# V2AI/Det3D

Measured on NVIDIA H100. Metric: point-clouds/sec SECOND SpMiddleFHD @20k pts, higher is better.
Workload: dtype f32

## Files before the change

### det3d_b200/csrc/spconv16_sm90.cu

```cuda
#include "epilogue16.cuh"

namespace d3b {

constexpr int kOsTileM = 128;
constexpr int kOsKc = 64;
constexpr int kOsABytes = kOsTileM * 128;

template <int COUT, int PLANES = 2>
struct OsCfg {
  static constexpr int kSlotHalves = 2 * COUT * kOsKc;
  static constexpr int kBBytes = PLANES * COUT * 128;
  static constexpr int kStageBytes = PLANES * kOsABytes + kBBytes;
  static constexpr int kStages = COUT >= 128 ? 3 : 4;
  static constexpr int kGroups = kStages;
  static constexpr int kMathWarps = 8;
  static constexpr int kGatherWarp0 = kMathWarps;
  static constexpr int kGroupThreads = 64;
  static constexpr int kThreads = 32 * (kGatherWarp0 + 2 * kGroups);
  static constexpr int kPassN = COUT >= 128 ? 64 : COUT;
  static constexpr int kSmemBytes = kStages * kStageBytes + 1024  + 256  + 32 * kOsTileM * 4;
};

template <int PLANES>
__device__ __forceinline__ bool epilogue16(float (&v)[16], const Epi16& e, size_t row_off, int col, __half* out_hi,
                                           __half* out_lo, float* out_f32) {
#pragma unroll
  for (int q = 0; q < 16; ++q) v[q] *= e.acc_scale;
  if (e.bias) {
#pragma unroll
    for (int q = 0; q < 16; q += 4) {
      const float4 b = __ldg(reinterpret_cast<const float4*>(e.bias + col + q));
      v[q] += b.x; v[q + 1] += b.y; v[q + 2] += b.z; v[q + 3] += b.w;
    }
  }
  if (e.scale) {
#pragma unroll
    for (int q = 0; q < 16; q += 4) {
      const float4 s = __ldg(reinterpret_cast<const float4*>(e.scale + col + q));
      const float4 t = __ldg(reinterpret_cast<const float4*>(e.shift + col + q));
      v[q] = fmaf(v[q], s.x, t.x); v[q + 1] = fmaf(v[q + 1], s.y, t.y);
      v[q + 2] = fmaf(v[q + 2], s.z, t.z); v[q + 3] = fmaf(v[q + 3], s.w, t.w);
    }
  }
  if (e.res_hi) {
#pragma unroll
    for (int q = 0; q < 16; q += 8) {
      if constexpr (PLANES == 2) {
        const uint4 h = __ldg(reinterpret_cast<const uint4*>(e.res_hi + row_off + col + q));
        const uint4 l = __ldg(reinterpret_cast<const uint4*>(e.res_lo + row_off + col + q));
        const uint32_t hw[4] = {h.x, h.y, h.z, h.w}, lw[4] = {l.x, l.y, l.z, l.w};
#pragma unroll
        for (int j = 0; j < 4; ++j) {
          const float2 fh = __half22float2(*reinterpret_cast<const __half2*>(&hw[j]));
          const float2 fl = __half22float2(*reinterpret_cast<const __half2*>(&lw[j]));
          v[q + 2 * j] += fh.x + fl.x;
          v[q + 2 * j + 1] += fh.y + fl.y;
        }
      } else {
        const uint4 h = __ldg(reinterpret_cast<const uint4*>(e.res_hi + row_off + col + q));
        const uint32_t hw[4] = {h.x, h.y, h.z, h.w};
#pragma unroll
        for (int j = 0; j < 4; ++j) {
          const float2 fh = __half22float2(*reinterpret_cast<const __half2*>(&hw[j]));
          v[q + 2 * j] += fh.x;
          v[q + 2 * j + 1] += fh.y;
        }
      }
    }
  }
  bool ovf = false;
  if (e.relu) {
#pragma unroll
    for (int q = 0; q < 16; ++q) v[q] = fmaxf(v[q], 0.f);
  }
  if (out_hi && PLANES == 2) {
    uint32_t hi[8], lo[8];
#pragma unroll
    for (int q = 0; q < 16; q += 2) ovf |= split_pack2(v[q], v[q + 1], hi[q >> 1], lo[q >> 1]);
    uint4* ph = reinterpret_cast<uint4*>(out_hi + row_off + col);
    uint4* pl = reinterpret_cast<uint4*>(out_lo + row_off + col);
    ph[0] = make_uint4(hi[0], hi[1], hi[2], hi[3]);
    ph[1] = make_uint4(hi[4], hi[5], hi[6], hi[7]);
    pl[0] = make_uint4(lo[0], lo[1], lo[2], lo[3]);
    pl[1] = make_uint4(lo[4], lo[5], lo[6], lo[7]);
  }
  if (out_hi && PLANES == 1) {
    uint32_t hi[8];
#pragma unroll
    for (int q = 0; q < 16; q += 2) {
      hi[q >> 1] = pack_half2(__float2half_rn(v[q]), __float2half_rn(v[q + 1]));
      ovf |= f16_out_of_range(v[q]) | f16_out_of_range(v[q + 1]);
    }
    uint4* ph = reinterpret_cast<uint4*>(out_hi + row_off + col);
    ph[0] = make_uint4(hi[0], hi[1], hi[2], hi[3]);
    ph[1] = make_uint4(hi[4], hi[5], hi[6], hi[7]);
  }
  if (out_f32) {
    float4* pf = reinterpret_cast<float4*>(out_f32 + row_off + col);
#pragma unroll
    for (int q = 0; q < 16; q += 4) pf[q >> 2] = make_float4(v[q], v[q + 1], v[q + 2], v[q + 3]);
  }
  return ovf;
}

template <int PLANES>
__device__ __forceinline__ bool epilogue2(float v0, float v1, const Epi16& e, size_t row_off, int col, __half* out_hi,
                                          __half* out_lo, float* out_f32) {
  v0 *= e.acc_scale;
  v1 *= e.acc_scale;
  v0 = fmaf(v0, e.corr, v0);
  v1 = fmaf(v1, e.corr, v1);
  if (e.bias) {
    const float2 b = __ldg(reinterpret_cast<const float2*>(e.bias + col));
    v0 += b.x; v1 += b.y;
  }
  if (e.scale) {
    const float2 s = __ldg(reinterpret_cast<const float2*>(e.scale + col));
    const float2 t = __ldg(reinterpret_cast<const float2*>(e.shift + col));
    v0 = fmaf(v0, s.x, t.x); v1 = fmaf(v1, s.y, t.y);
  }
  if (e.res_hi) {
    const float2 r = load_pair16<PLANES>(e.res_hi, e.res_lo, row_off + col);
    v0 += r.x;
    v1 += r.y;
  }
  if (e.relu) { v0 = fmaxf(v0, 0.f); v1 = fmaxf(v1, 0.f); }
  bool ovf = false;
  if (out_hi) ovf = store_pair16<PLANES>(v0, v1, out_hi, out_lo, row_off + col);
  if (out_f32) *reinterpret_cast<float2*>(out_f32 + row_off + col) = make_float2(v0, v1);
  return ovf;
}

__host__ __device__ inline int os16_pack(int c_in, int k_vol) {
  return k_vol > 1 && (c_in == 16 || c_in == 32) ? kOsKc / c_in : 1;
}
__device__ __forceinline__ unsigned int os16_slot_mask(unsigned int offset_mask, int pack) {
  if (pack == 1) return offset_mask;
  unsigned int r = 0u;
  const unsigned int grp = (1u << pack) - 1u;
  for (int p = 0; p * pack < 32; ++p) r |= ((offset_mask >> (p * pack)) & grp) ? (1u << p) : 0u;
  return r;
}

template <int COUT, int PLANES>
__device__ __forceinline__ void spconv_os16_body(
    const __half* __restrict__ in_hi, const __half* __restrict__ in_lo, const int* __restrict__ nbr,
    const unsigned int* __restrict__ tile_mask, const int* __restrict__ n_out_p, int out_cap, int c_in, int n_kb, int pack,
    int k_vol, const __half* __restrict__ packed, const Epi16& epi, __half* __restrict__ out_hi, __half* __restrict__ out_lo,
    float* __restrict__ out_f32, int* __restrict__ overflow) {
  using Cfg = OsCfg<COUT, PLANES>;
  extern __shared__ uint8_t smem_raw[];
  const uint32_t smem_base = (smem_u32(smem_raw) + 1023u) & ~1023u;
  uint8_t* smem_gen = smem_raw + (smem_base - smem_u32(smem_raw));
  const uint32_t bar_base = smem_base + Cfg::kStages * Cfg::kStageBytes;
  auto full_bar = [&](int s) { return bar_base + 8u * s; };
  auto empty_bar = [&](int s) { return bar_base + 8u * (Cfg::kStages + s); };
  const uint32_t nbr_bar = bar_base + 8u * (2 * Cfg::kStages);
  int* koff_s = reinterpret_cast<int*>(smem_gen + Cfg::kStages * Cfg::kStageBytes + 128);
  int* nbr_s = reinterpret_cast<int*>(smem_gen + Cfg::kStages * Cfg::kStageBytes + 256);

  D3B_CTA_MARK(0, epi.seq);
  pdl_launch_dependents();
  const int warp = threadIdx.x >> 5, lane = threadIdx.x & 31;
  const int n_out = min(*n_out_p, out_cap);
  const int n_tiles = (n_out + kOsTileM - 1) / kOsTileM;
  const int c_eff = c_in * pack;

  if (threadIdx.x == 0) {
    for (int s = 0; s < Cfg::kStages; ++s) {
      mbar_init(full_bar(s), Cfg::kGroupThreads + 1);
      mbar_init(empty_bar(s), Cfg::kMathWarps);
    }
    mbar_init(nbr_bar, 1);
    asm volatile("fence.mbarrier_init.release.cluster;" ::: "memory");
  }
  __syncthreads();

  if (warp < Cfg::kMathWarps) {
    pdl_wait_prior_grid();
    const int wg = warp >> 2, wq = warp & 3;
    bool ovf = false;
    uint32_t it = 0;
    for (int tile = blockIdx.x; tile < n_tiles; tile += gridDim.x) {
      const unsigned int smask = os16_slot_mask(tile_mask[tile], pack);
      const int n_slots = __popc(smask) * n_kb;
      float acc[COUT / 2];
#pragma unroll
      for (int q = 0; q < COUT / 2; ++q) acc[q] = 0.f;
      for (int j = 0; j < n_slots; ++j, ++it) {
        const int kb = n_kb == 1 ? 0 : j % n_kb;
        const int s = it % Cfg::kStages;
        const uint32_t ph = (it / Cfg::kStages) & 1u;
        const int n_ks = min(kOsKc / 16, (c_eff - kb * kOsKc + 15) / 16);
        if (warp == 0 && lane == 0) D3B_STAMP(6, it);
        D3B_WAIT(full_bar(s), ph, 3);
        const uint32_t a_hi = smem_base + s * Cfg::kStageBytes + wg * 8192u;
        const uint32_t a_lo = a_hi + kOsABytes;
        const uint32_t b_hi = smem_base + s * Cfg::kStageBytes + PLANES * kOsABytes;
        const uint32_t b_lo = b_hi + COUT * 128;
#pragma unroll
        for (int np = 0; np < COUT / Cfg::kPassN; ++np) {
          float part[Cfg::kPassN / 2];
          const uint32_t nb = np * Cfg::kPassN * 128;
          gmma_fence();
#pragma unroll
          for (int ks = 0; ks < kOsKc / 16; ++ks) {
            const uint32_t adv = ks * 32;
            if constexpr (PLANES == 2) {
              wgmma_f16<Cfg::kPassN>(part, gmma_desc_sw128(a_lo + adv), gmma_desc_sw128(b_hi + nb + adv), ks > 0 ? 1u : 0u);
              wgmma_f16<Cfg::kPassN>(part, gmma_desc_sw128(a_hi + adv), gmma_desc_sw128(b_lo + nb + adv), 1u);
              wgmma_f16<Cfg::kPassN>(part, gmma_desc_sw128(a_hi + adv), gmma_desc_sw128(b_hi + nb + adv), 1u);
            } else {
              wgmma_f16<Cfg::kPassN>(part, gmma_desc_sw128(a_hi + adv), gmma_desc_sw128(b_hi + nb + adv), ks > 0 ? 1u : 0u);
            }
          }
          gmma_commit();
          gmma_wait();
          gmma_fence_regs(part);
#pragma unroll
          for (int q = 0; q < Cfg::kPassN / 2; ++q) acc[np * Cfg::kPassN / 2 + q] += part[q];
        }
        __syncwarp();
        if (lane == 0) mbar_arrive(empty_bar(s));
        if (warp == 0 && lane == 0) D3B_STAMP(7, it);
      }
#pragma unroll
      for (int h = 0; h < 2; ++h) {
        const int o = tile * kOsTileM + wg * 64 + wq * 16 + (lane >> 2) + 8 * h;
        if (o >= n_out) continue;
#pragma unroll
        for (int jn = 0; jn < COUT / 8; ++jn)
          ovf |= epilogue2<PLANES>(acc[4 * jn + 2 * h], acc[4 * jn + 2 * h + 1], epi, (size_t)o * COUT, jn * 8 + 2 * (lane & 3),
                           out_hi, out_lo, out_f32);
      }
    }
    if (ovf && overflow) atomicOr(overflow, 1);
  } else {
    const int gw = warp - Cfg::kGatherWarp0;
    const int group = gw >> 1, wq = gw & 1;
    const int g = lane >> 3, c = lane & 7;
    const bool issues_tma = (wq == 0 && lane == 0);
    const int ptid = threadIdx.x - 32 * Cfg::kGatherWarp0;
    const int cpo = 8 / pack;
    const int sub = c / cpo;
    const int c_src = c - sub * cpo;
    uint32_t it0 = 0;
    uint32_t tile_count = 0;
    const bool bulk_nbr = (out_cap & 3) == 0;
    for (int tile = blockIdx.x; tile < n_tiles; tile += gridDim.x) {
      const int row0 = tile * kOsTileM;
      const unsigned int mask = os16_slot_mask(tile_mask[tile], pack);
      const int n_off = __popc(mask);
      const int n_slots = n_off * n_kb;

      asm volatile("bar.sync 1, %0;" ::"r"(Cfg::kGroupThreads * Cfg::kGroups) : "memory");
      if (ptid < 32) {
        unsigned int m = mask;
        for (int t = ptid; t > 0; --t) m &= m - 1;
        const int k = __ffs(m) - 1;
        if (ptid < n_off) koff_s[ptid] = k;
        __syncwarp();
        const int rows = min(kOsTileM, out_cap - row0);
        const int e_slot = ptid / pack;
        const int k_src = ptid < n_off * pack ? koff_s[e_slot] * pack + (ptid - e_slot * pack) : k_vol;
        const bool valid = k_src < k_vol;
        const unsigned int vm = __ballot_sync(0xffffffffu, valid);
        if (bulk_nbr && vm != 0u && ptid == 0) mbar_arrive_expect_tx(nbr_bar, (uint32_t)(__popc(vm) * rows * 4));
        __syncwarp();
        if (bulk_nbr && valid)
          tma_bulk_g2s(smem_u32(nbr_s + ptid * kOsTileM), nbr + (size_t)k_src * out_cap + row0, (uint32_t)(rows * 4), nbr_bar);
      }
      if (bulk_nbr) {
        if (n_off > 0) D3B_WAIT(nbr_bar, tile_count & 1u, 5);
      } else {
        asm volatile("bar.sync 1, %0;" ::"r"(Cfg::kGroupThreads * Cfg::kGroups) : "memory");
#pragma unroll 8
        for (int idx = ptid; idx < n_off * pack * kOsTileM; idx += Cfg::kGroupThreads * Cfg::kGroups) {
          const int r = idx & 127, e = idx >> 7;
          const int k_src = koff_s[e / pack] * pack + e % pack;
          nbr_s[idx] = k_src < k_vol ? __ldg(nbr + (size_t)k_src * out_cap + min(row0 + r, out_cap - 1)) : -1;
        }
      }
      asm volatile("bar.sync 1, %0;" ::"r"(Cfg::kGroupThreads * Cfg::kGroups) : "memory");
      if (n_off > 0) ++tile_count;
      if (tile == (int)blockIdx.x) pdl_wait_prior_grid();

      for (int j = (int)((group + Cfg::kGroups - (it0 % Cfg::kGroups)) % Cfg::kGroups); j < n_slots; j += Cfg::kGroups) {
        const int n = j / n_kb, kb = j - n * n_kb;
        const int ch = pack > 1 ? c_src * 8 : kb * kOsKc + c * 8;
        const uint32_t it = it0 + (uint32_t)j;
        const int s = it % Cfg::kStages;
        const uint32_t ph = (it / Cfg::kStages) & 1u;
        if (issues_tma) D3B_STAMP(0, it);
        D3B_WAIT(empty_bar(s), ph ^ 1u, 1);
        if (issues_tma) D3B_STAMP(1, it);
        const uint32_t stage = smem_base + s * Cfg::kStageBytes;
        if (issues_tma) {
          mbar_arrive_expect_tx(full_bar(s), Cfg::kBBytes);
          tma_bulk_g2s(stage + PLANES * kOsABytes, packed + ((size_t)koff_s[n] * n_kb + kb) * Cfg::kSlotHalves, Cfg::kBBytes,
                       full_bar(s));
        }
        {
          const int row_base = wq * 64 + g * 16;
          const int4* idx4 = reinterpret_cast<const int4*>(nbr_s + (n * pack + sub) * kOsTileM + row_base);
          const bool col_live = pack > 1 ? koff_s[n] * pack + sub < k_vol : ch < c_in;
#pragma unroll
          for (int q4 = 0; q4 < 4; ++q4) {
            const int4 iv = idx4[q4];
            const int srcs[4] = {iv.x, iv.y, iv.z, iv.w};
#pragma unroll
            for (int u = 0; u < 4; ++u) {
              const int row = row_base + q4 * 4 + u;
              const bool live = srcs[u] >= 0 && col_live && row0 + row < n_out;
              const size_t off = live ? (size_t)srcs[u] * c_in + ch : 0;
              const uint32_t dst = stage + sw128_offset(row, c);
              cp_async16(dst, in_hi + off, live ? 16u : 0u);
              if constexpr (PLANES == 2) cp_async16(dst + kOsABytes, in_lo + off, live ? 16u : 0u);
            }
          }
        }
        if (issues_tma) D3B_STAMP(2, it);
        cp_async_wait_all();
        if (issues_tma) D3B_STAMP(3, it);
        fence_proxy_async();
        mbar_arrive(full_bar(s));
      }
      it0 += (uint32_t)n_slots;
    }
  }
  D3B_CTA_MARK(1, epi.seq);
}

template <int COUT>
__global__ void __launch_bounds__(OsCfg<COUT>::kThreads, 1)
spconv_os16_kernel(const __half* __restrict__ in_hi, const __half* __restrict__ in_lo, const int* __restrict__ nbr,
                   const unsigned int* __restrict__ tile_mask, const int* __restrict__ n_out_p, int out_cap, int c_in,
                   int n_kb, int pack, int k_vol, const __half* __restrict__ packed, Epi16 epi, __half* __restrict__ out_hi,
                   __half* __restrict__ out_lo, float* __restrict__ out_f32, int* __restrict__ overflow) {
  spconv_os16_body<COUT, 2>(in_hi, in_lo, nbr, tile_mask, n_out_p, out_cap, c_in, n_kb, pack, k_vol, packed, epi, out_hi,
                            out_lo, out_f32, overflow);
}

template <int COUT>
__global__ void __launch_bounds__(OsCfg<COUT, 1>::kThreads, 1)
spconv_os16_f16_kernel(const __half* __restrict__ in_hi, const __half* __restrict__ in_lo, const int* __restrict__ nbr,
                       const unsigned int* __restrict__ tile_mask, const int* __restrict__ n_out_p, int out_cap, int c_in,
                       int n_kb, int pack, int k_vol, const __half* __restrict__ packed, Epi16 epi,
                       __half* __restrict__ out_hi, __half* __restrict__ out_lo, float* __restrict__ out_f32,
                       int* __restrict__ overflow) {
  spconv_os16_body<COUT, 1>(in_hi, in_lo, nbr, tile_mask, n_out_p, out_cap, c_in, n_kb, pack, k_vol, packed, epi, out_hi,
                            out_lo, out_f32, overflow);
}

template <int COUT, int PLANES>
__device__ __forceinline__ void spconv_first16_body(
    const float* __restrict__ feat_in, const int* __restrict__ nbr, const int* __restrict__ n_out_p, int out_cap, int c_in,
    int in_ld, int k_vol, const float* __restrict__ weight, Epi16 epi, __half* __restrict__ out_hi,
    __half* __restrict__ out_lo, float* __restrict__ out_f32, int* __restrict__ overflow) {
  extern __shared__ float w_s[];
  for (int i = threadIdx.x; i < k_vol * c_in * COUT; i += blockDim.x) w_s[i] = weight[i];
  __syncthreads();
  constexpr int kParts = COUT / 16;
  constexpr int kSub = 4;
  constexpr int kMaxK = 8;
  const int n_out = min(*n_out_p, out_cap);
  const long long items = (long long)n_out * kParts;
  const long long items_pad = (items + 7) / 8 * 8;
  bool ovf = false;
  for (long long e = (long long)blockIdx.x * blockDim.x + threadIdx.x; e < items_pad * kSub; e += (long long)gridDim.x * blockDim.x) {
    const long long item = e / kSub;
    const int sub = (int)(e % kSub);
    const bool on = item < items;
    const int o = on ? (int)(item / kParts) : 0, col = (int)(item % kParts) * 16;
    int src[kMaxK];
#pragma unroll
    for (int t = 0; t < kMaxK; ++t) {
      const int k = sub + t * kSub;
      src[t] = (on && k < k_vol) ? __ldg(nbr + (size_t)k * out_cap + o) : -1;
    }
    float acc[16];
#pragma unroll
    for (int q = 0; q < 16; ++q) acc[q] = 0.f;
#pragma unroll
    for (int t = 0; t < kMaxK; ++t) {
      if (src[t] < 0) continue;
      const int k = sub + t * kSub;
      for (int ci = 0; ci < c_in; ++ci) {
        const float a = __ldg(feat_in + (size_t)src[t] * in_ld + ci);
        const float* w = w_s + ((size_t)k * c_in + ci) * COUT + col;
#pragma unroll
        for (int q = 0; q < 16; ++q) acc[q] = fmaf(a, w[q], acc[q]);
      }
    }
#pragma unroll
    for (int q = 0; q < 16; ++q) {
      acc[q] += __shfl_xor_sync(0xffffffffu, acc[q], 1);
      acc[q] += __shfl_xor_sync(0xffffffffu, acc[q], 2);
    }
    if (on && sub == 0) ovf |= epilogue16<PLANES>(acc, epi, (size_t)o * COUT, col, out_hi, out_lo, out_f32);
  }
  if (ovf && overflow) atomicOr(overflow, 1);
}

template <int COUT>
__global__ void __launch_bounds__(256)
spconv_first16_kernel(const float* __restrict__ feat_in, const int* __restrict__ nbr, const int* __restrict__ n_out_p,
                      int out_cap, int c_in, int in_ld, int k_vol, const float* __restrict__ weight, Epi16 epi,
                      __half* __restrict__ out_hi, __half* __restrict__ out_lo, float* __restrict__ out_f32,
                      int* __restrict__ overflow) {
  spconv_first16_body<COUT, 2>(feat_in, nbr, n_out_p, out_cap, c_in, in_ld, k_vol, weight, epi, out_hi, out_lo, out_f32,
                               overflow);
}

template <int COUT>
__global__ void __launch_bounds__(256)
spconv_first16_f16_kernel(const float* __restrict__ feat_in, const int* __restrict__ nbr, const int* __restrict__ n_out_p,
                          int out_cap, int c_in, int in_ld, int k_vol, const float* __restrict__ weight, Epi16 epi,
                          __half* __restrict__ out_hi, __half* __restrict__ out_lo, float* __restrict__ out_f32,
                          int* __restrict__ overflow) {
  spconv_first16_body<COUT, 1>(feat_in, nbr, n_out_p, out_cap, c_in, in_ld, k_vol, weight, epi, out_hi, out_lo, out_f32,
                               overflow);
}

__global__ void __launch_bounds__(256)
pack_weight16_kernel(const float* __restrict__ w, int c_in, int c_out, int k_vol, int n_slots_k, int n_kb, int pack,
                     float w_mul, __half* __restrict__ packed) {
  const long long total = (long long)n_slots_k * n_kb * 2 * c_out * kOsKc;
  for (long long e = (long long)blockIdx.x * blockDim.x + threadIdx.x; e < total; e += (long long)gridDim.x * blockDim.x) {
    long long t = e;
    const int cc = (int)(t % kOsKc); t /= kOsKc;
    const int n = (int)(t % c_out); t /= c_out;
    const int part = (int)(t % 2); t /= 2;
    const int kb = (int)(t % n_kb); t /= n_kb;
    int k = (int)t;
    int ci = kb * kOsKc + cc;
    if (pack > 1) { k = k * pack + cc / c_in; ci = cc % c_in; }
    const float x = (ci < c_in && k < k_vol) ? w[((size_t)k * c_in + ci) * c_out + n] * w_mul : 0.0f;
    k = (int)t;
    __half hi, lo;
    split_f16(x, hi, lo);
    const size_t tile = (((size_t)k * n_kb + kb) * 2 + part) * (size_t)(c_out * kOsKc);
    const uint32_t off = sw128_offset(n, cc >> 3) + (cc & 7) * 2;
    packed[tile + off / 2] = part == 0 ? hi : lo;
  }
}

template <int PLANES>
__global__ void __launch_bounds__(256)
split16_kernel(const float* __restrict__ x, long long n, __half* __restrict__ hi, __half* __restrict__ lo,
               int* __restrict__ overflow) {
  bool ovf = false;
  for (long long e = (long long)blockIdx.x * blockDim.x + threadIdx.x; e < n; e += (long long)gridDim.x * blockDim.x) {
    ovf |= store16p<PLANES>(x[e], hi + e, lo + e);
  }
  if (ovf && overflow) atomicOr(overflow, 1);
}

template <int PLANES>
__global__ void __launch_bounds__(256)
merge16_kernel(const __half* __restrict__ hi, const __half* __restrict__ lo, long long n, float* __restrict__ x) {
  for (long long e = (long long)blockIdx.x * blockDim.x + threadIdx.x; e < n; e += (long long)gridDim.x * blockDim.x) {
    if constexpr (PLANES == 2) x[e] = __half2float(hi[e]) + __half2float(lo[e]);
    else x[e] = __half2float(hi[e]);
  }
}

template <int PLANES>
__global__ void __launch_bounds__(256)
sparse_to_bev16_kernel(const __half* __restrict__ in_hi, const __half* __restrict__ in_lo, const float* __restrict__ in_f32,
                       const int* __restrict__ coors, const int* __restrict__ n_rows, int row_cap, int C, int D, int H,
                       int W, int B, __half* __restrict__ out_hi, __half* __restrict__ out_lo, int* __restrict__ overflow) {
  const int n = min(*n_rows, row_cap);
  const long long total = (long long)n * C;
  for (long long e = (long long)blockIdx.x * blockDim.x + threadIdx.x; e < total; e += (long long)gridDim.x * blockDim.x) {
    const int r = (int)(e / C), c = (int)(e - (long long)r * C);
    const int4 q = *reinterpret_cast<const int4*>(coors + (size_t)r * 4);
    if ((unsigned)q.x >= (unsigned)B || (unsigned)q.y >= (unsigned)D || (unsigned)q.z >= (unsigned)H ||
        (unsigned)q.w >= (unsigned)W)
      continue;
    const size_t dst = (((size_t)q.x * H + q.z) * W + q.w) * ((size_t)C * D) + (size_t)c * D + q.y;
    if (in_f32) {
      if (store16p<PLANES>(in_f32[e], out_hi + dst, out_lo + dst) && overflow) {
        if ((__activemask() & ((1u << (threadIdx.x & 31)) - 1u)) == 0u) atomicOr(overflow, 1);
      }
    } else {
      out_hi[dst] = in_hi[e];
      if constexpr (PLANES == 2) out_lo[dst] = in_lo[e];
    }
  }
}

static bool os16_shape_ok(int c_in, int c_out) {
  const bool cin_ok = c_in >= 8 && c_in <= 512 && c_in % 8 == 0;
  const bool cout_ok = c_out == 16 || c_out == 32 || c_out == 64 || c_out == 128;
  return cin_ok && cout_ok;
}

static Epi16 epi_of(const d3b_conv16_params* p) {
  Epi16 e;
  e.bias = p->bias; e.scale = p->scale; e.shift = p->shift;
  e.res_hi = (const __half*)p->residual_hi; e.res_lo = (const __half*)p->residual_lo;
  e.acc_scale = p->acc_scale; e.relu = p->relu;
  e.corr = 0.f;
  static std::atomic<int> launch_seq{0};
  e.seq = launch_seq.fetch_add(1, std::memory_order_relaxed);
  return e;
}

template <int COUT, int PLANES>
static int launch_os16(const d3b_conv16_params* p, const int32_t* nbr, const uint32_t* tile_mask, const int32_t* n_out,
                       int32_t out_cap, cudaStream_t stream) {
  using Cfg = OsCfg<COUT, PLANES>;
  constexpr auto kernel = PLANES == 2 ? spconv_os16_kernel<COUT> : spconv_os16_f16_kernel<COUT>;
  static SmemOptIn optin;
  D3B_CUDA(ensure_dynamic_smem(kernel, Cfg::kSmemBytes, optin));
  const int n_tiles = div_up(out_cap, kOsTileM);
  const int grid = n_tiles < kNumSMs ? (n_tiles > 0 ? n_tiles : 1) : kNumSMs;
  const int pack = os16_pack(p->c_in, p->k_vol);
  const int n_kb = pack > 1 ? 1 : (p->c_in + kOsKc - 1) / kOsKc;
  Epi16 epi = epi_of(p);
  epi.corr = trunc_correction(p->c_in * pack, PLANES == 2 ? 3 : 1);
  D3B_CUDA(launch_maybe_pdl(kernel, dim3(grid), dim3(Cfg::kThreads), Cfg::kSmemBytes, stream,
                            (const __half*)p->in_hi, (const __half*)p->in_lo, (const int*)nbr, (const unsigned int*)tile_mask,
                            (const int*)n_out, (int)out_cap, (int)p->c_in, n_kb, pack, (int)p->k_vol,
                            (const __half*)p->weight_packed, epi,
                            (__half*)p->out_hi, (__half*)p->out_lo, p->out_f32, (int*)p->overflow));
  D3B_LAUNCH_CHECK();
  return D3B_OK;
}

template <int COUT, int PLANES>
static int launch_first16(const d3b_conv16_params* p, const int32_t* nbr, const int32_t* n_out, int32_t out_cap,
                          cudaStream_t stream) {
  constexpr auto kernel = PLANES == 2 ? spconv_first16_kernel<COUT> : spconv_first16_f16_kernel<COUT>;
  const size_t smem = (size_t)p->k_vol * p->c_in * COUT * sizeof(float);
  static SmemOptIn optin;
  D3B_REQUIRE(smem <= 160 * 1024, "first-layer sparse conv: weights (%zu bytes) do not fit in shared memory", smem);
  D3B_CUDA(ensure_dynamic_smem(kernel, smem, optin));
  const int grid = grid_for((long long)out_cap * (COUT / 16) * 4, 256, 8);
  const int in_ld = p->in_f32_ld ? p->in_f32_ld : p->c_in;
  kernel<<<grid, 256, smem, stream>>>(p->in_f32, nbr, n_out, out_cap, p->c_in, in_ld, p->k_vol, p->weight,
                                                         epi_of(p), (__half*)p->out_hi, (__half*)p->out_lo, p->out_f32,
                                                         p->overflow);
  D3B_LAUNCH_CHECK();
  return D3B_OK;
}

}

using namespace d3b;

extern "C" size_t d3b_conv16_packed_weight_halves(int32_t c_in, int32_t c_out, int32_t k_vol) {
  if (c_in < 1 || c_in > 512 || k_vol < 1 || k_vol > 32) return 0;
  if (!(c_out == 16 || c_out == 32 || c_out == 64 || c_out == 128)) return 0;
  const int pack = os16_pack(c_in, k_vol);
  const int n_kb = pack > 1 ? 1 : (c_in + kOsKc - 1) / kOsKc;
  return (size_t)div_up(k_vol, pack) * n_kb * 2 * c_out * kOsKc;
}

extern "C" int d3b_conv16_pack_weight(const float* weight_dev, int32_t c_in, int32_t c_out, int32_t k_vol,
                                      int32_t w_exp, void* packed_dev, void* stream_) {
  cudaStream_t stream = (cudaStream_t)stream_;
  D3B_REQUIRE(weight_dev && packed_dev, "d3b_conv16_pack_weight: null argument");
  D3B_REQUIRE(w_exp >= -60 && w_exp <= 60, "d3b_conv16_pack_weight: w_exp %d outside [-60, 60]", w_exp);
  const size_t n = d3b_conv16_packed_weight_halves(c_in, c_out, k_vol);
  if (n == 0) {
    set_error("d3b_conv16_pack_weight: unsupported C_in=%d C_out=%d k_vol=%d", c_in, c_out, k_vol);
    return D3B_ERR_UNSUPPORTED;
  }
  const int pack = os16_pack(c_in, k_vol);
  const int n_kb = pack > 1 ? 1 : (c_in + kOsKc - 1) / kOsKc;
  pack_weight16_kernel<<<grid_for((long long)n, 256), 256, 0, stream>>>(weight_dev, c_in, c_out, k_vol, div_up(k_vol, pack),
                                                                        n_kb, pack, ldexpf(1.0f, w_exp), (__half*)packed_dev);
  D3B_LAUNCH_CHECK();
  return D3B_OK;
}

extern "C" int d3b_sparse_conv16(const int32_t* nbr, const uint32_t* tile_mask, const int32_t* n_out, int32_t out_cap,
                                 const d3b_conv16_params* p, void* stream_) {
  cudaStream_t stream = (cudaStream_t)stream_;
  D3B_REQUIRE(nbr && n_out && p, "d3b_sparse_conv16: null argument");
  D3B_REQUIRE(p->k_vol >= 1 && p->k_vol <= 32 && out_cap >= 0, "d3b_sparse_conv16: bad shape (k_vol %d)", p->k_vol);
  D3B_REQUIRE(p->out_hi || p->out_f32, "d3b_sparse_conv16: give out_hi (+ out_lo) and/or out_f32");
  D3B_REQUIRE((p->scale == nullptr) == (p->shift == nullptr), "d3b_sparse_conv16: scale and shift go together");
  PlanePairs pp;
  pp.add(p->in_f32 ? nullptr : p->in_hi, p->in_lo);
  pp.add(p->out_hi, p->out_lo);
  pp.add(p->residual_hi, p->residual_lo);
  D3B_REQUIRE(pp.consistent(),
              "d3b_sparse_conv16: give in_lo, out_lo and residual_lo with their hi planes (FP16x3) or none of them "
              "(single-pass FP16); got in_lo %s, out_lo %s, residual_lo %s",
              p->in_lo ? "set" : "NULL", p->out_lo ? "set" : "NULL", p->residual_lo ? "set" : "NULL");
  const bool two = pp.planes() == 2;
  if (out_cap == 0) return D3B_OK;
  if (p->in_f32) {
    D3B_REQUIRE(p->weight && p->c_in >= 1 && p->c_in <= 16, "d3b_sparse_conv16: fp32-input layers need weight and C_in <= 16");
    D3B_REQUIRE(p->in_f32_ld == 0 || p->in_f32_ld >= p->c_in, "d3b_sparse_conv16: in_f32_ld %d < C_in %d", p->in_f32_ld,
                p->c_in);
    switch (p->c_out) {
      case 16: return two ? launch_first16<16, 2>(p, nbr, n_out, out_cap, stream) : launch_first16<16, 1>(p, nbr, n_out, out_cap, stream);
      case 32: return two ? launch_first16<32, 2>(p, nbr, n_out, out_cap, stream) : launch_first16<32, 1>(p, nbr, n_out, out_cap, stream);
      case 64: return two ? launch_first16<64, 2>(p, nbr, n_out, out_cap, stream) : launch_first16<64, 1>(p, nbr, n_out, out_cap, stream);
      default:
        set_error("d3b_sparse_conv16: fp32-input layer with C_out=%d (16/32/64 built)", p->c_out);
        return D3B_ERR_UNSUPPORTED;
    }
  }
  D3B_REQUIRE(tile_mask && p->in_hi && p->weight_packed, "d3b_sparse_conv16: null planes / tile_mask / packed weights");
  if (!os16_shape_ok(p->c_in, p->c_out)) {
    set_error("d3b_sparse_conv16: unsupported C_in=%d C_out=%d", p->c_in, p->c_out);
    return D3B_ERR_UNSUPPORTED;
  }
  switch (p->c_out) {
    case 16: return two ? launch_os16<16, 2>(p, nbr, tile_mask, n_out, out_cap, stream) : launch_os16<16, 1>(p, nbr, tile_mask, n_out, out_cap, stream);
    case 32: return two ? launch_os16<32, 2>(p, nbr, tile_mask, n_out, out_cap, stream) : launch_os16<32, 1>(p, nbr, tile_mask, n_out, out_cap, stream);
    case 64: return two ? launch_os16<64, 2>(p, nbr, tile_mask, n_out, out_cap, stream) : launch_os16<64, 1>(p, nbr, tile_mask, n_out, out_cap, stream);
    default: return two ? launch_os16<128, 2>(p, nbr, tile_mask, n_out, out_cap, stream) : launch_os16<128, 1>(p, nbr, tile_mask, n_out, out_cap, stream);
  }
}

extern "C" int d3b_split16(const float* x, int64_t n, void* hi, void* lo, int32_t* overflow, void* stream_) {
  cudaStream_t stream = (cudaStream_t)stream_;
  D3B_REQUIRE(n >= 0 && (n == 0 || (x && hi)), "d3b_split16: null argument");
  if (n == 0) return D3B_OK;
  if (lo) split16_kernel<2><<<grid_for(n, 256), 256, 0, stream>>>(x, n, (__half*)hi, (__half*)lo, overflow);
  else split16_kernel<1><<<grid_for(n, 256), 256, 0, stream>>>(x, n, (__half*)hi, nullptr, overflow);
  D3B_LAUNCH_CHECK();
  return D3B_OK;
}

extern "C" int d3b_merge16(const void* hi, const void* lo, int64_t n, float* x, void* stream_) {
  cudaStream_t stream = (cudaStream_t)stream_;
  D3B_REQUIRE(n >= 0 && (n == 0 || (x && hi)), "d3b_merge16: null argument");
  if (n == 0) return D3B_OK;
  if (lo) merge16_kernel<2><<<grid_for(n, 256), 256, 0, stream>>>((const __half*)hi, (const __half*)lo, n, x);
  else merge16_kernel<1><<<grid_for(n, 256), 256, 0, stream>>>((const __half*)hi, nullptr, n, x);
  D3B_LAUNCH_CHECK();
  return D3B_OK;
}

extern "C" int d3b_sparse_to_bev16(const void* in_hi, const void* in_lo, const float* in_f32, const int32_t* coors,
                                   const int32_t* n_rows, int32_t row_cap, int32_t channels, const int32_t spatial[3],
                                   int32_t batch, void* out_hi, void* out_lo, int32_t* overflow, void* stream_) {
  cudaStream_t stream = (cudaStream_t)stream_;
  D3B_REQUIRE(coors && n_rows && spatial && out_hi, "d3b_sparse_to_bev16: null argument");
  D3B_REQUIRE((in_f32 != nullptr) != (in_hi != nullptr), "d3b_sparse_to_bev16: give fp32 rows OR planes");
  PlanePairs pp;
  pp.add(in_hi, in_lo);
  pp.add(out_hi, out_lo);
  D3B_REQUIRE(pp.consistent(),
              "d3b_sparse_to_bev16: give in_lo (plane rows) and out_lo together (FP16x3) or neither (single-pass FP16); "
              "got in_lo %s, out_lo %s", in_lo ? "set" : "NULL", out_lo ? "set" : "NULL");
  D3B_REQUIRE(channels >= 1 && batch >= 1 && row_cap >= 0, "d3b_sparse_to_bev16: bad shape");
  if (row_cap == 0) return D3B_OK;
  const int grid = grid_for((long long)row_cap * channels, 256);
  if (pp.planes() == 2)
    sparse_to_bev16_kernel<2><<<grid, 256, 0, stream>>>((const __half*)in_hi, (const __half*)in_lo, in_f32, coors, n_rows,
                                                        row_cap, channels, spatial[0], spatial[1], spatial[2], batch,
                                                        (__half*)out_hi, (__half*)out_lo, overflow);
  else
    sparse_to_bev16_kernel<1><<<grid, 256, 0, stream>>>((const __half*)in_hi, nullptr, in_f32, coors, n_rows, row_cap,
                                                        channels, spatial[0], spatial[1], spatial[2], batch,
                                                        (__half*)out_hi, nullptr, overflow);
  D3B_LAUNCH_CHECK();
  return D3B_OK;
}

#ifdef D3B_SOFT_TIMEOUT
extern "C" int d3b_debug_fault_spconv16(unsigned int* host8) {
  cudaError_t e = cudaMemcpyFromSymbol(host8, d3b::g_d3b_fault, 32);
  unsigned int zeros[8] = {0};
  if (e == cudaSuccess) e = cudaMemcpyToSymbol(d3b::g_d3b_fault, zeros, 32);
  return (int)e;
}
extern "C" int d3b_debug_cta_ns_spconv16(unsigned long long* host4096) {
  return (int)cudaMemcpyFromSymbol(host4096, d3b::g_d3b_cta_ns, sizeof(unsigned long long) * 4096);
}
extern "C" int d3b_debug_cta_clk_spconv16(long long* host4096) {
  return (int)cudaMemcpyFromSymbol(host4096, d3b::g_d3b_cta_clk, sizeof(long long) * 4096);
}
extern "C" int d3b_debug_trace_spconv16(long long* host, int clear) {
  cudaError_t e = cudaMemcpyFromSymbol(host, d3b::g_d3b_trace, sizeof(long long) * 16 * 512);
  if (e == cudaSuccess && clear) {
    static long long zeros[16 * 512];
    e = cudaMemcpyToSymbol(d3b::g_d3b_trace, zeros, sizeof(zeros));
  }
  return (int)e;
}
#endif
```

Baseline: 1010.

## Compact live rows per kernel offset and fold partial sums into shared memory

The gather warps now build a compacted list of live output rows for each kernel-offset slot and pack only those rows into the A tile. Each math warpgroup runs WGMMA only on 64-row blocks that contain live rows, alternating blocks between the two groups. Results are scattered into a shared-memory fp32 accumulator indexed through the row map, with a swizzle to reduce bank conflicts. This skips tensor-core and gather work on empty neighbour rows, but adds shared-memory read-modify-write folds, a spin-wait counter that orders the folds, and a large shared-memory tail that may reduce the pipeline stage count.

```diff
diff --git a/det3d_b200/csrc/spconv16_sm90.cu b/det3d_b200/csrc/spconv16_sm90.cu
--- a/det3d_b200/csrc/spconv16_sm90.cu
+++ b/det3d_b200/csrc/spconv16_sm90.cu
@@ -11,15 +11,24 @@
   static constexpr int kSlotHalves = 2 * COUT * kOsKc;
   static constexpr int kBBytes = PLANES * COUT * 128;
   static constexpr int kStageBytes = PLANES * kOsABytes + kBBytes;
-  static constexpr int kStages = COUT >= 128 ? 3 : 4;
+  static constexpr int kSumsOff = 256 + 32 * kOsTileM * 4 + 4 * kOsTileM + 128;
+  static constexpr int kTailBytes = kSumsOff + kOsTileM * COUT * 4;
+  static constexpr int kStages = (232448 - 1024 - kTailBytes) / kStageBytes < 4 ? (232448 - 1024 - kTailBytes) / kStageBytes : 4;
   static constexpr int kGroups = kStages;
   static constexpr int kMathWarps = 8;
   static constexpr int kGatherWarp0 = kMathWarps;
   static constexpr int kGroupThreads = 64;
   static constexpr int kThreads = 32 * (kGatherWarp0 + 2 * kGroups);
   static constexpr int kPassN = COUT >= 128 ? 64 : COUT;
-  static constexpr int kSmemBytes = kStages * kStageBytes + 1024  + 256  + 32 * kOsTileM * 4;
+  static constexpr int kSmemBytes = kStages * kStageBytes + 1024  + kTailBytes;
+  static_assert(kStages >= 2, "sparse conv: the pipeline needs two stages");
 };
+
+template <int COUT>
+__device__ __forceinline__ int os16_sum_idx(int row, int col) {
+  const int x = COUT == 16 ? ((row >> 1) & 1) << 3 : (row & 3) << 3;
+  return row * COUT + (col ^ x);
+}
 
 template <int PLANES>
 __device__ __forceinline__ bool epilogue16(float (&v)[16], const Epi16& e, size_t row_off, int col, __half* out_hi,
@@ -158,13 +167,16 @@
   const uint32_t nbr_bar = bar_base + 8u * (2 * Cfg::kStages);
   int* koff_s = reinterpret_cast<int*>(smem_gen + Cfg::kStages * Cfg::kStageBytes + 128);
   int* nbr_s = reinterpret_cast<int*>(smem_gen + Cfg::kStages * Cfg::kStageBytes + 256);
+  uint8_t* map_s = smem_gen + Cfg::kStages * Cfg::kStageBytes + 256 + 32 * kOsTileM * 4;
+  int* nlive_s = reinterpret_cast<int*>(map_s + 4 * kOsTileM);
+  int* fold_cnt = nlive_s + 4;
+  float* sums = reinterpret_cast<float*>(smem_gen + Cfg::kStages * Cfg::kStageBytes + Cfg::kSumsOff);
 
   D3B_CTA_MARK(0, epi.seq);
   pdl_launch_dependents();
   const int warp = threadIdx.x >> 5, lane = threadIdx.x & 31;
   const int n_out = min(*n_out_p, out_cap);
   const int n_tiles = (n_out + kOsTileM - 1) / kOsTileM;
-  const int c_eff = c_in * pack;
 
   if (threadIdx.x == 0) {
     for (int s = 0; s < Cfg::kStages; ++s) {
@@ -172,6 +184,7 @@
       mbar_init(empty_bar(s), Cfg::kMathWarps);
     }
     mbar_init(nbr_bar, 1);
+    *fold_cnt = 0;
     asm volatile("fence.mbarrier_init.release.cluster;" ::: "memory");
   }
   __syncthreads();
@@ -179,66 +192,112 @@
   if (warp < Cfg::kMathWarps) {
     pdl_wait_prior_grid();
     const int wg = warp >> 2, wq = warp & 3;
+    auto consumers_sync = [] { asm volatile("bar.sync 2, %0;" ::"r"(32 * Cfg::kMathWarps) : "memory"); };
+    auto wait_folds = [&](int n_warps) {
+      for (uint32_t spin = 0; *reinterpret_cast<volatile int*>(fold_cnt) < n_warps; ++spin) {
+        if (spin > (1u << 28)) __trap();
+      }
+      __threadfence_block();
+    };
+    for (int i = threadIdx.x; i < kOsTileM * COUT; i += 32 * Cfg::kMathWarps) sums[i] = 0.f;
+    consumers_sync();
     bool ovf = false;
     uint32_t it = 0;
+    int units = 0;
     for (int tile = blockIdx.x; tile < n_tiles; tile += gridDim.x) {
       const unsigned int smask = os16_slot_mask(tile_mask[tile], pack);
       const int n_slots = __popc(smask) * n_kb;
-      float acc[COUT / 2];
-#pragma unroll
-      for (int q = 0; q < COUT / 2; ++q) acc[q] = 0.f;
       for (int j = 0; j < n_slots; ++j, ++it) {
-        const int kb = n_kb == 1 ? 0 : j % n_kb;
         const int s = it % Cfg::kStages;
         const uint32_t ph = (it / Cfg::kStages) & 1u;
-        const int n_ks = min(kOsKc / 16, (c_eff - kb * kOsKc + 15) / 16);
         if (warp == 0 && lane == 0) D3B_STAMP(6, it);
         D3B_WAIT(full_bar(s), ph, 3);
-        const uint32_t a_hi = smem_base + s * Cfg::kStageBytes + wg * 8192u;
-        const uint32_t a_lo = a_hi + kOsABytes;
-        const uint32_t b_hi = smem_base + s * Cfg::kStageBytes + PLANES * kOsABytes;
-        const uint32_t b_lo = b_hi + COUT * 128;
-#pragma unroll
-        for (int np = 0; np < COUT / Cfg::kPassN; ++np) {
-          float part[Cfg::kPassN / 2];
-          const uint32_t nb = np * Cfg::kPassN * 128;
+        const int n_live = nlive_s[s];
+        const int n_blk = (n_live + 63) >> 6;
+        const int blk = (wg ^ units) & 1;
+        const bool mine = blk < n_blk;
+        float part[COUT / Cfg::kPassN][Cfg::kPassN / 2];
+        int rows[2];
+        if (mine) {
+#pragma unroll
+          for (int h = 0; h < 2; ++h) {
+            const int p = blk * 64 + wq * 16 + (lane >> 2) + 8 * h;
+            rows[h] = p < n_live ? map_s[s * kOsTileM + p] : -1;
+          }
+          const uint32_t a_hi = smem_base + s * Cfg::kStageBytes + blk * 8192u;
+          const uint32_t a_lo = a_hi + kOsABytes;
+          const uint32_t b_hi = smem_base + s * Cfg::kStageBytes + PLANES * kOsABytes;
+          const uint32_t b_lo = b_hi + COUT * 128;
           gmma_fence();
 #pragma unroll
-          for (int ks = 0; ks < kOsKc / 16; ++ks) {
-            const uint32_t adv = ks * 32;
-            if constexpr (PLANES == 2) {
-              wgmma_f16<Cfg::kPassN>(part, gmma_desc_sw128(a_lo + adv), gmma_desc_sw128(b_hi + nb + adv), ks > 0 ? 1u : 0u);
-              wgmma_f16<Cfg::kPassN>(part, gmma_desc_sw128(a_hi + adv), gmma_desc_sw128(b_lo + nb + adv), 1u);
-              wgmma_f16<Cfg::kPassN>(part, gmma_desc_sw128(a_hi + adv), gmma_desc_sw128(b_hi + nb + adv), 1u);
-            } else {
-              wgmma_f16<Cfg::kPassN>(part, gmma_desc_sw128(a_hi + adv), gmma_desc_sw128(b_hi + nb + adv), ks > 0 ? 1u : 0u);
+          for (int np = 0; np < COUT / Cfg::kPassN; ++np) {
+            const uint32_t nb = np * Cfg::kPassN * 128;
+#pragma unroll
+            for (int ks = 0; ks < kOsKc / 16; ++ks) {
+              const uint32_t adv = ks * 32;
+              if constexpr (PLANES == 2) {
+                wgmma_f16<Cfg::kPassN>(part[np], gmma_desc_sw128(a_lo + adv), gmma_desc_sw128(b_hi + nb + adv), ks > 0 ? 1u : 0u);
+                wgmma_f16<Cfg::kPassN>(part[np], gmma_desc_sw128(a_hi + adv), gmma_desc_sw128(b_lo + nb + adv), 1u);
+                wgmma_f16<Cfg::kPassN>(part[np], gmma_desc_sw128(a_hi + adv), gmma_desc_sw128(b_hi + nb + adv), 1u);
+              } else {
+                wgmma_f16<Cfg::kPassN>(part[np], gmma_desc_sw128(a_hi + adv), gmma_desc_sw128(b_hi + nb + adv), ks > 0 ? 1u : 0u);
+              }
             }
           }
           gmma_commit();
           gmma_wait();
-          gmma_fence_regs(part);
-#pragma unroll
-          for (int q = 0; q < Cfg::kPassN / 2; ++q) acc[np * Cfg::kPassN / 2 + q] += part[q];
+#pragma unroll
+          for (int np = 0; np < COUT / Cfg::kPassN; ++np) gmma_fence_regs(part[np]);
         }
         __syncwarp();
         if (lane == 0) mbar_arrive(empty_bar(s));
         if (warp == 0 && lane == 0) D3B_STAMP(7, it);
-      }
+        if (mine) {
+          wait_folds(4 * units);
+#pragma unroll
+          for (int h = 0; h < 2; ++h) {
+            if (rows[h] < 0) continue;
+#pragma unroll
+            for (int np = 0; np < COUT / Cfg::kPassN; ++np)
+#pragma unroll
+              for (int jn = 0; jn < Cfg::kPassN / 8; ++jn) {
+                float2* d = reinterpret_cast<float2*>(
+                    sums + os16_sum_idx<COUT>(rows[h], np * Cfg::kPassN + jn * 8 + 2 * (lane & 3)));
+                float2 v = *d;
+                v.x += part[np][4 * jn + 2 * h];
+                v.y += part[np][4 * jn + 2 * h + 1];
+                *d = v;
+              }
+          }
+          __syncwarp();
+          if (lane == 0) {
+            __threadfence_block();
+            atomicAdd(fold_cnt, 1);
+          }
+        }
+        units += n_blk;
+      }
+      wait_folds(4 * units);
 #pragma unroll
       for (int h = 0; h < 2; ++h) {
-        const int o = tile * kOsTileM + wg * 64 + wq * 16 + (lane >> 2) + 8 * h;
-        if (o >= n_out) continue;
-#pragma unroll
-        for (int jn = 0; jn < COUT / 8; ++jn)
-          ovf |= epilogue2<PLANES>(acc[4 * jn + 2 * h], acc[4 * jn + 2 * h + 1], epi, (size_t)o * COUT, jn * 8 + 2 * (lane & 3),
-                           out_hi, out_lo, out_f32);
-      }
+        const int r = wg * 64 + wq * 16 + (lane >> 2) + 8 * h;
+        const int o = tile * kOsTileM + r;
+#pragma unroll
+        for (int jn = 0; jn < COUT / 8; ++jn) {
+          float2* d = reinterpret_cast<float2*>(sums + os16_sum_idx<COUT>(r, jn * 8 + 2 * (lane & 3)));
+          const float2 v = *d;
+          *d = make_float2(0.f, 0.f);
+          if (o < n_out)
+            ovf |= epilogue2<PLANES>(v.x, v.y, epi, (size_t)o * COUT, jn * 8 + 2 * (lane & 3), out_hi, out_lo, out_f32);
+        }
+      }
+      consumers_sync();
     }
     if (ovf && overflow) atomicOr(overflow, 1);
   } else {
     const int gw = warp - Cfg::kGatherWarp0;
     const int group = gw >> 1, wq = gw & 1;
-    const int g = lane >> 3, c = lane & 7;
+    const int c = lane & 7, pg = wq * 4 + (lane >> 3);
     const bool issues_tma = (wq == 0 && lane == 0);
     const int ptid = threadIdx.x - 32 * Cfg::kGatherWarp0;
     const int cpo = 8 / pack;
@@ -300,23 +359,40 @@
           tma_bulk_g2s(stage + PLANES * kOsABytes, packed + ((size_t)koff_s[n] * n_kb + kb) * Cfg::kSlotHalves, Cfg::kBBytes,
                        full_bar(s));
         }
+        uint32_t live_bits[4];
+        int n_live = 0, p_warp = 0;
+#pragma unroll
+        for (int q = 0; q < 4; ++q) {
+          const int row = q * 32 + lane;
+          bool live = false;
+          if (row0 + row < n_out)
+            for (int m = 0; m < pack; ++m)
+              live |= koff_s[n] * pack + m < k_vol && nbr_s[(n * pack + m) * kOsTileM + row] >= 0;
+          live_bits[q] = __ballot_sync(0xffffffffu, live);
+          if (q == 2 * wq) p_warp = n_live;
+          n_live += __popc(live_bits[q]);
+        }
+        uint8_t* map = map_s + s * kOsTileM;
+#pragma unroll
+        for (int qq = 0; qq < 2; ++qq) {
+          const uint32_t bits = wq ? live_bits[2 + qq] : live_bits[qq];
+          if ((bits >> lane) & 1u) map[p_warp + __popc(bits & ((1u << lane) - 1u))] = (uint8_t)((2 * wq + qq) * 32 + lane);
+          p_warp += __popc(bits);
+        }
+        if (issues_tma) nlive_s[s] = n_live;
+        asm volatile("bar.sync %0, %1;" ::"r"(3 + group), "r"(Cfg::kGroupThreads) : "memory");
         {
-          const int row_base = wq * 64 + g * 16;
-          const int4* idx4 = reinterpret_cast<const int4*>(nbr_s + (n * pack + sub) * kOsTileM + row_base);
+          const int* idx = nbr_s + (n * pack + sub) * kOsTileM;
           const bool col_live = pack > 1 ? koff_s[n] * pack + sub < k_vol : ch < c_in;
-#pragma unroll
-          for (int q4 = 0; q4 < 4; ++q4) {
-            const int4 iv = idx4[q4];
-            const int srcs[4] = {iv.x, iv.y, iv.z, iv.w};
-#pragma unroll
-            for (int u = 0; u < 4; ++u) {
-              const int row = row_base + q4 * 4 + u;
-              const bool live = srcs[u] >= 0 && col_live && row0 + row < n_out;
-              const size_t off = live ? (size_t)srcs[u] * c_in + ch : 0;
-              const uint32_t dst = stage + sw128_offset(row, c);
-              cp_async16(dst, in_hi + off, live ? 16u : 0u);
-              if constexpr (PLANES == 2) cp_async16(dst + kOsABytes, in_lo + off, live ? 16u : 0u);
-            }
+          const int p_end = (n_live + 63) & ~63;
+#pragma unroll 4
+          for (int p = pg; p < p_end; p += 8) {
+            const int src = p < n_live ? idx[map[p]] : -1;
+            const bool live = src >= 0 && col_live;
+            const size_t off = live ? (size_t)src * c_in + ch : 0;
+            const uint32_t dst = stage + sw128_offset(p, c);
+            cp_async16(dst, in_hi + off, live ? 16u : 0u);
+            if constexpr (PLANES == 2) cp_async16(dst + kOsABytes, in_lo + off, live ? 16u : 0u);
           }
         }
         if (issues_tma) D3B_STAMP(2, it);
```

Result: slower. 900.3, median of 6 (-10.8%).
